# flanglet/kanzi-cpp

Hardware: AMD Instinct MI355X
Metric: encode+decode MB/s on the synthetic stand-in for silesia.tar (bit-exact) (higher is better)
Workload: dtype u8

## Files before the change

kanzi-cpp_amd/csrc/bwt_fwd.hip:

```cpp
#include "common.hpp"
#include "stages.hpp"
#include "bwt_common.hpp"

#include <cstdlib>
#include <cstring>
#include <algorithm>
#include <cmath>
#include "prims.hpp"
#include <chrono>
#include <vector>

namespace knz {

constexpr u32 SM_TS = 1792;
constexpr u32 SM_WIN = 2048;
constexpr u32 SM_G = 256;
constexpr u32 MED_CAP = 8192;
constexpr u32 SUPER_CAP = 8192;
constexpr int GATHER_THREADS = 512;
constexpr u32 LARGE_OS_MIN = 1000000;
constexpr u32 NO_BIT = 0x7FFFFFFFu;

struct FwdView {
    const u32* base;
// ... 1030 lines not shown
        if (mLab != oldLab) lab_set(v, gp, L.blkBase, mLab, oldLab);
    }
    u32 surv = 0;
    if (tid == 0) {
        if (less != 0) atomicOr(&v.gnew[mStart >> 5], 1u << (mStart & 31));
        if (c > SM_G) v.medStage[mStart >> 8] = make_uint2(mStart, c);
        else if (c > 1) surv = 1;
    }
    if ((u32)tid < nOth) {
        const u32 t = (u32)tid;
        const u32 key = L.oK[t];
        u32 hd = t, e = t + 1;
        while (hd > 0 && L.oK[hd - 1] == key) hd--;
        while (e < nOth && L.oK[e] == key) e++;
        const u32 size = e - hd;
        const u32 shift = (t < less) ? 0u : c;
        const u32 slot = gs + t + shift, hdSlot = gs + hd + shift;
        const u32 relO = rel - shift;
        const u32 lab = (size <= SM_G) ? hdSlot : ((oldLab >= hdSlot && oldLab < hdSlot + size) ? oldLab : hdSlot + (size >> 1));
        (void)relO;
        const u32 gp = L.oV[t];
        v.SA[slot] = gp;
        if (lab != oldLab) lab_set(v, gp, L.blkBase, lab, oldLab);
        if (t == hd) {
            if (hdSlot != gs) atomicOr(&v.gnew[hdSlot >> 5], 1u << (hdSlot & 31));
            if (size > SM_G) v.medStage[hdSlot >> 8] = make_uint2(hdSlot, size);
            else if (size > 1) surv = 1;
        }
    }
    if (__ballot(surv != 0) != 0 && (tid & 63) == 0) v.counters[0] = 1;
}

template <int THREADS, int ROWS>
__global__ __launch_bounds__(THREADS, (THREADS >= 1024 ? 4 : THREADS / 128)) void k_bwt_f_sort_medium(FwdView v, const uint2* __restrict__ desc, u32 nDesc, int npass, u32 minLen,
                                                               uint2* __restrict__ medNext, uint2* __restrict__ largeNext, const uint2* __restrict__ descInfo,
                                                               uint4* __restrict__ superList)
{
    constexpr int WAVES = THREADS / 64;
    constexpr u32 CAP = (u32)ROWS * THREADS;
    __shared__ MedLds<THREADS, ROWS> L;
    const int tid = (int)threadIdx.x, lane = tid & 63, wave = tid >> 6;
    const unsigned long long ltMask = (lane == 0) ? 0ull : (~0ull >> (64 - lane));

    for (u32 g = blockIdx.x; g < nDesc; g += gridDim.x) {
        const uint2 d = desc[g];
        const u32 gs = d.x, n = d.y;
        if (n <= minLen || n > CAP) continue;
        const uint2 info = descInfo[g];
        {
            u32 k[ROWS], p[ROWS];
#pragma unroll
            for (int r = 0; r < ROWS; r++) { const u32 i = (u32)tid + (u32)r * THREADS; k[r] = 0; p[r] = 0; if (i < n) { k[r] = v.K[gs + i]; p[r] = v.SA[gs + i]; } }
#pragma unroll
            for (int r = 0; r < ROWS; r++) { const u32 i = (u32)tid + (u32)r * THREADS; if (i < n) { L.oK[i] = k[r]; L.oV[i] = p[r]; } }
        }
        __syncthreads();
        if (tid == 0) { L.oldLab = info.y; L.blkBase = info.x; }
        const u32 ka = L.oK[n >> 2], kb = L.oK[n >> 1], kc = L.oK[(n >> 2) * 3];
        const u32 m = (ka == kc) ? ka : kb;
        u32 c = 0;
        for (u32 i = (u32)tid; i < n; i += THREADS) c += (L.oK[i] == m) ? 1u : 0u;
        c = med_block_sum(L, c);
        if (c < n && 2 * c >= n && n <= SUPER_CAP && m == info.y - info.x + 1u) {
            if (tid == 0) { const u32 at = atomicAdd(&v.counters[7], 1u); superList[at] = make_uint4(gs, n, info.x, info.y); }
            __syncthreads();
            continue;
        }
        if (c < n) {
            if (2 * c >= n) {
                const int R = (int)((n + THREADS - 1) / THREADS);
                const u32 waveBase = (u32)wave * (u32)R * 64u;
                u32 key[ROWS], val[ROWS], pos[ROWS];
                u32 runO = 0, runE = 0;
#pragma unroll
                for (int r = 0; r < ROWS; r++) {
                    key[r] = m; val[r] = 0; pos[r] = 0xFFFFFFFFu;
                    if (r < R) {
                        const u32 idx = waveBase + (u32)r * 64u + (u32)lane;
                        const bool valid = idx < n;
                        if (valid) { key[r] = L.oK[idx]; val[r] = L.oV[idx]; }
                        const bool oth = valid && key[r] != m, same = valid && key[r] == m;
                        const unsigned long long bo = __ballot(oth), be = __ballot(same);
                        if (oth) pos[r] = runO + (u32)__popcll(bo & ltMask);
                        if (same) pos[r] = 0x80000000u | (runE + (u32)__popcll(be & ltMask));
                        runO += (u32)__popcll(bo);
                        runE += (u32)__popcll(be);
                    }
                }
                if (lane == 0) { L.wtot[wave] = runO; L.wtot2[wave] = runE; }
                __syncthreads();
                u32 baseO = 0, baseE = 0, nOth = 0;
                for (int w = 0; w < WAVES; w++) { if (w < wave) { baseO += L.wtot[w]; baseE += L.wtot2[w]; } nOth += L.wtot[w]; }
#pragma unroll
                for (int r = 0; r < ROWS; r++) {
                    if (r < R && pos[r] != 0xFFFFFFFFu) {
                        const u32 at = (pos[r] & 0x80000000u) ? (nOth + baseE + (pos[r] & 0x7FFFFFFFu)) : (baseO + pos[r]);
                        L.oK[at] = key[r];
                        L.oV[at] = val[r];
                    }
                }
                __syncthreads();
                if (nOth <= (u32)THREADS) {
                    u32 kk = 0, vv = 0, at = 0;
                    if ((u32)tid < nOth) {
                        kk = L.oK[tid]; vv = L.oV[tid];
                        for (u32 j = 0; j < nOth; j++) { const u32 kj = L.oK[j]; at += (kj < kk || (kj == kk && j < (u32)tid)) ? 1u : 0u; }
                    }
                    __syncthreads();
                    if ((u32)tid < nOth) { L.oK[at] = kk; L.oV[at] = vv; }
                    __syncthreads();
                    u32 lessQ = 0;
                    if ((u32)tid < nOth) lessQ = (L.oK[tid] < m) ? 1u : 0u;
                    lessQ = med_block_sum(L, lessQ);
                    if (tid == 0) { L.oldLab = info.y; L.blkBase = info.x; }
                    __syncthreads();
                    med_majority_write_back<THREADS, ROWS>(L, v, gs, n, nOth, c, lessQ, m);
                    __syncthreads();
                    continue;
                } else {
                    med_radix_sort<THREADS, ROWS>(L, nOth, npass);
                }
                u32 less = 0;
                for (u32 i = (u32)tid; i < nOth; i += THREADS) less += (L.oK[i] < m) ? 1u : 0u;
                less = med_block_sum(L, less);
#pragma unroll
                for (int k = 0; k < ROWS; k++) {
                    const u32 i = (u32)tid + (u32)k * THREADS;
                    if (i < n) { key[k] = L.oK[i]; val[k] = L.oV[i]; }
                }
                __syncthreads();
#pragma unroll
                for (int k = 0; k < ROWS; k++) {
                    const u32 i = (u32)tid + (u32)k * THREADS;
                    if (i < n) {
                        const u32 at = (i < less) ? i : (i < nOth ? i + c : less + (i - nOth));
                        L.oK[at] = key[k];
                        L.oV[at] = val[k];
                    }
                }
                __syncthreads();
            } else {
                med_radix_sort<THREADS, ROWS>(L, n, npass);
            }
// ... 109 lines not shown
            cm = wave_max(cm);
            if (lane == 0 && cm) atomicMax(&sCmax, cm);
        }
        __syncthreads();
        const u32 cmax = sCmax;
        const u32 trBits = bitlen_u32(nEnds ? nEnds - 1 : 0), hiBits = bitlen_u32(2u * cmax + 1u);
        u32 fk[ROWS];
#pragma unroll
        for (int r = 0; r < ROWS; r++) {
            const u32 i = (u32)tid + (u32)r * THREADS;
            fk[r] = 0;
            if (i < n) { const u32 hiKey = (tail[r] < m) ? cc[r] : (2u * cmax + 1u - cc[r]); fk[r] = (hiKey << trBits) | (u32)trEnd[e[r]]; }
        }
        __syncthreads();
#pragma unroll
        for (int r = 0; r < ROWS; r++) { const u32 i = (u32)tid + (u32)r * THREADS; if (i < n) { L.oK[i] = fk[r]; L.oV[i] = i; } }
        __syncthreads();
        med_radix_sort<THREADS, ROWS>(L, n, (int)((hiBits + trBits + 7) / 8));
        {
            u32 p[ROWS];
#pragma unroll
            for (int r = 0; r < ROWS; r++) { const u32 i = (u32)tid + (u32)r * THREADS; p[r] = 0; if (i < n) p[r] = v.SA[gs + L.oV[i]]; }
            __syncthreads();
#pragma unroll
            for (int r = 0; r < ROWS; r++) { const u32 i = (u32)tid + (u32)r * THREADS; if (i < n) L.oV[i] = p[r]; }
        }
        __syncthreads();
        med_write_back<THREADS, ROWS>(L, v, gs, n, medNext, largeNext);
        __syncthreads();
    }
}

constexpr u32 PROBE_PMAX = 2048;
__global__ __launch_bounds__(256) void k_bwt_f_probe_scan(FwdView v, const uint2* __restrict__ desc, u32 depth, const u32* __restrict__ rtbits, u32* __restrict__ cand)
{
    const u32 nDesc = v.counters[1];
    for (u32 g = blockIdx.x * 256 + threadIdx.x; g < nDesc; g += gridDim.x * 256) {
        const uint2 d = desc[g];
        const u32 gs = d.x, n = d.y;
        if (n <= SM_G || n > SUPER_CAP) continue;
        if (rtbits != nullptr && ((rtbits[gs >> 5] >> (gs & 31)) & 1u)) continue;
        const u32 a0 = v.SA[gs + (n >> 1) - 2], a1 = v.SA[gs + (n >> 1) - 1], a2 = v.SA[gs + (n >> 1)], a3 = v.SA[gs + (n >> 1) + 1];
        const u32 pd = a2 - a1;
        if ((a1 - a0 == pd) && (a3 - a2 == pd) && (pd > depth) && (pd <= 2048u) && ((pd & (pd - 1)) != 0)) cand[atomicAdd(&v.counters[14], 1u)] = g;
    }
}

__global__ __launch_bounds__(512, 4) void k_bwt_f_probe(BwtView bv, FwdView v, uint2* __restrict__ desc, const u32* __restrict__ cand, u32 nCand, u32 depth, uint2* __restrict__ medNext,
                                                        uint2* __restrict__ largeNext, u32* __restrict__ ovr, u32* __restrict__ rtbits)
{
    constexpr int THREADS = 512, ROWS = 16;
    constexpr u32 CAP = (u32)ROWS * THREADS;
    __shared__ MedLds<THREADS, ROWS> L;
    __shared__ u32 patw[PROBE_PMAX / 4];
    u8* pat = reinterpret_cast<u8*>(patw);
    __shared__ u32 sInfo[4];
    const int tid = (int)threadIdx.x;
    for (u32 cg = blockIdx.x; cg < nCand; cg += gridDim.x) {
        const u32 g = cand[cg];
        const uint2 d = desc[g];
        const u32 gs = d.x, n = d.y;
        bool take = n > SM_G && n <= CAP;
        __syncthreads();
        if (take) {
            for (u32 i = (u32)tid; i < n; i += THREADS) L.oV[i] = v.SA[gs + i];
            if (tid == 0) {
                const int b = find_block(v.base, v.nBlocks, gs);
                sInfo[0] = v.base[b]; sInfo[1] = v.base[b + 1]; sInfo[3] = (u32)b;
            }
        }
        __syncthreads();
        u32 P = 0, pr = 0;
        if (take) {
            pr = L.oV[n >> 1];
            P = pr - L.oV[(n >> 1) - 1];
            take = P > depth && P <= PROBE_PMAX && pr + P <= sInfo[1];
        }
        if (take) {
            u32 c = 0;
            for (u32 i = (u32)tid; i + 1 < n; i += THREADS) c += (L.oV[i + 1] - L.oV[i] == P) ? 1u : 0u;
            c = med_block_sum(L, c);
            take = 2 * c >= n;
        }
        if (!take) continue;
        const u32 bb = sInfo[0], be = sInfo[1];
        const u8* t = bv.src[sInfo[3]];
        for (u32 j = (u32)tid; j < P; j += THREADS) pat[j] = ldg<u8>(t + (pr - bb + j));
        if (tid == 0) sInfo[2] = lab_cur(v, pr, sInfo[0]);
        __syncthreads();
        constexpr u32 MID = 1u << 21;
        u32 nEq = 0, nBelow = 0;
        for (u32 i = (u32)tid; i < n; i += THREADS) {
            const u32 q0 = L.oV[i] - bb;
            u32 l = depth;
            if ((depth & 3u) == 0) {
                const u32* pw = patw;
                while (l + 16 <= P && q0 + l + 20 <= be - bb) {
                    const uintptr_t ad = reinterpret_cast<uintptr_t>(t + q0 + l);
                    const u8* w = reinterpret_cast<const u8*>(ad & ~(uintptr_t)3);
                    const u32 sh = (u32)(ad & 3) * 8;
                    const u32 w0 = ldg<u32>(w), w1 = ldg<u32>(w + 4), w2 = ldg<u32>(w + 8), w3 = ldg<u32>(w + 12), w4 = ldg<u32>(w + 16);
                    const u32 x0 = sh ? ((w0 >> sh) | (w1 << (32 - sh))) : w0, x1 = sh ? ((w1 >> sh) | (w2 << (32 - sh))) : w1;
                    const u32 x2 = sh ? ((w2 >> sh) | (w3 << (32 - sh))) : w2, x3 = sh ? ((w3 >> sh) | (w4 << (32 - sh))) : w3;
                    const u32 d0 = x0 ^ pw[l >> 2], d1 = x1 ^ pw[(l >> 2) + 1], d2 = x2 ^ pw[(l >> 2) + 2], d3 = x3 ^ pw[(l >> 2) + 3];
                    if ((d0 | d1 | d2 | d3) != 0) break;
                    l += 16;
                }
            }
            u32 code = MID;
            while (l < P) {
                if (q0 + l >= be - bb) { code = l * 512u; break; }
                const u32 x = ldg<u8>(t + q0 + l), y = pat[l];
                if (x != y) { code = (x < y) ? (l * 512u + x + 1u) : (MID + 1u + (P - l) * 512u + x + 1u); break; }
                l++;
            }
            L.oK[i] = code;
            nEq += (code == MID) ? 1u : 0u;
            nBelow += (code < MID) ? 1u : 0u;
        }
        nEq = med_block_sum(L, nEq);
        nBelow = med_block_sum(L, nBelow);
        if (2 * nEq < n) continue;
        if (tid == 0) { L.oldLab = sInfo[2]; L.blkBase = sInfo[0]; desc[g].y = 0; }
        med_radix_sort<THREADS, ROWS>(L, n, 3);
        med_write_back<THREADS, ROWS>(L, v, gs, n, medNext, largeNext);
        for (u32 i = (u32)tid; i < n; i += THREADS) {
            const u32 code = L.oK[i];
            const u32 lshare = (code == MID) ? P : ((code < MID) ? (code >> 9) : (P - ((code - MID - 1u) >> 9))) + 1u;
            ovr[gs + i] = lshare;
            atomicOr(&rtbits[(gs + i) >> 5], 1u << ((gs + i) & 31));
        }
    }
}

__global__ __launch_bounds__(1024) void k_bwt_f_large_prefix(const uint2* __restrict__ desc, u32 nDesc, u32* __restrict__ loff, const u32* __restrict__ base, int nBlocks,
                                                             u32* __restrict__ lbase)
{
    __shared__ u32 part[1024];
    const u32 per = (nDesc + 1023) / 1024;
    const u32 lo = threadIdx.x * per, hi = (lo + per < nDesc) ? lo + per : nDesc;
    u32 sum = 0;
    for (u32 i = lo; i < hi; i++) { sum += desc[i].y; lbase[i] = base[find_block(base, nBlocks, desc[i].x)]; }
    part[threadIdx.x] = sum;
    __syncthreads();
    if (threadIdx.x == 0) { u32 run = 0; for (int t = 0; t < 1024; t++) { const u32 x = part[t]; part[t] = run; run += x; } loff[nDesc] = run; }
    __syncthreads();
    u32 run = part[threadIdx.x];
    for (u32 i = lo; i < hi; i++) { loff[i] = run; run += desc[i].y; }
}

template <class KEY>
__global__ __launch_bounds__(256) void k_bwt_f_large_keys(FwdView v, const uint2* __restrict__ desc, u32 nDesc, const u32* __restrict__ loff,
                                                          u32 L, u32 h, int kbits, KEY* __restrict__ keys, u32* __restrict__ vals)
{
    const u32 j = blockIdx.x * 256 + threadIdx.x;
    if (j >= L) return;
    u32 lo = 0, hi = nDesc;
    while (hi - lo > 1) { const u32 mid = (lo + hi) >> 1; if (loff[mid] <= j) lo = mid; else hi = mid; }
    const uint2 d = desc[lo];
    const u32 slot = d.x + (j - loff[lo]);
    const int b = find_block(v.base, v.nBlocks, d.x);
    const u32 gp = v.SA[slot];
    u32 off = h;
// ... 398 lines not shown
            const u32 q = 4 * w + k;
            if (q >= qLo && q < qHi) {
                const u32 rr = q - qLo;
                const u32 r = rr + (rr >= r0 ? 1u : 0u);
                const u32 p = SA[bb + r] - bb;
                word |= (u32)s[p - 1] << (8 * k);
                have |= 1u << k;
            }
        }
        if (have == 0xF && al) reinterpret_cast<u32*>(d)[w] = word;
        else for (u32 k = 0; k < 4; k++) if ((have >> k) & 1) d[4 * w + k] = (u8)(word >> (8 * k));
    }
    if (blockIdx.x == 0 && threadIdx.x == 0) {
        d[hdr] = s[n - 1];
        const u32 st = n / (u32)chunks;
        const u32 step = ((u32)chunks * st == n) ? st : st + 1;
        const u32 logNbChunks = (u32)ilog2_u32((u32)chunks);
        d[0] = (u8)((logNbChunks << 2) | (pIndexSize - 1));
        u32 idx = 1;
        for (int k = 0; k < chunks; k++) {
            const u32 prim = lab_cur(fv, bb + (u32)k * step, bb) - bb;
            for (int sh = (int)(pIndexSize - 1) * 8; sh >= 0; sh -= 8) d[idx++] = (u8)(prim >> sh);
        }
        newLen[b] = hdr + n;
    }
}

__global__ __launch_bounds__(256) void k_bwt_f_med_flags(const uint2* __restrict__ stage, u32 nSlots, u32* __restrict__ flags)
{
    const u32 i = blockIdx.x * 256 + threadIdx.x;
    if (i < nSlots) flags[i] = stage[i].y ? 1u : 0u;
}

__global__ __launch_bounds__(256) void k_bwt_f_med_compact(uint2* __restrict__ stage, u32 nSlots, const u32* __restrict__ prefix, uint2* __restrict__ medNext)
{
    const u32 i = blockIdx.x * 256 + threadIdx.x;
    if (i >= nSlots) return;
    const uint2 d = stage[i];
    if (d.y) { medNext[prefix[i]] = d; stage[i] = make_uint2(0u, 0u); }
}

struct FwdTuning { int nsym; int noRunRound; int runFallback; int stats; int link; int plainLabels; int noPack; };
static FwdTuning& fwd_tuning()
{
    static FwdTuning t = [] {
        FwdTuning x; x.nsym = 0; x.noRunRound = 0; x.runFallback = 0; x.stats = 0; x.link = 1; x.plainLabels = 0; x.noPack = 0;
        if (getenv("KNZ_BWT_PLAIN_LABELS")) x.plainLabels = 1;
        if (getenv("KNZ_BWT_NO_PACK")) x.noPack = 1;
        if (const char* e = getenv("KNZ_BWT_LINK")) x.link = atoi(e);
        if (getenv("KNZ_BWT_STATS")) x.stats = 1;
        if (const char* e = getenv("KNZ_BWT_NSYM")) x.nsym = atoi(e);
        if (getenv("KNZ_BWT_NO_RUN_ROUND")) x.noRunRound = 1;
        if (getenv("KNZ_BWT_RUN_FALLBACK")) x.runFallback = 1;
        return x;
    }();
    return t;
}
int bwt_forward_tune(const char* key, int value)
{
    FwdTuning& t = fwd_tuning();
    if (!strcmp(key, "rs_onesweep")) { prims::rs_onesweep_knob().store(value); return 0; }
    if (!strcmp(key, "bwt_nsym")) t.nsym = value;
    else if (!strcmp(key, "bwt_no_run_round")) t.noRunRound = value;
    else if (!strcmp(key, "bwt_run_fallback")) t.runFallback = value;
    else if (!strcmp(key, "bwt_stats")) t.stats = value;
    else if (!strcmp(key, "bwt_link")) t.link = value;
// ... 138 lines not shown
        std::swap(kin, kout);
    }
    const u64* sortedKeys = kin;
    u64* keysFree = kout;
    u64* keysFree2 = const_cast<u64*>(sortedKeys);
    hipMemsetAsync(w.gbits, 0xFF, 4 * w.gbitsWords, s);
    hipMemsetAsync(w.gnew, 0, 4 * w.gbitsWords, s);
    hipMemsetAsync(w.counters, 0, 64, s);
    { KScope ks_("k_bwt_f_r0_flags"); hipLaunchKernelGGL(k_bwt_f_r0_flags, dim3((total + 256 * R0F_ROWS - 1) / (256 * R0F_ROWS)), dim3(256), 0, s, sortedKeys, w.base, st.nBlocks, total, nsym, pbits,
                                                         reinterpret_cast<unsigned long long*>(w.gbits)); }
    const u32 nWinP = (total + SM_TS - 1) / SM_TS;
    { KScope ks_("k_bwt_f_r0_winsum"); hipLaunchKernelGGL(k_bwt_f_r0_winsum, GRID1(nWinP), w.gbits, total, nWinP, w.t0, w.t2, SM_TS / 32); }
    { KScope ks_("k_bwt_f_scan_max"); prims::launch_scan<prims::SCAN_MAX_INCL>(s, w.t0, w.t1, nWinP, nullptr, w.scanTmp); }
    { KScope ks_("k_bwt_f_scan_min"); prims::launch_scan<prims::SCAN_MIN_INCL>(s, w.t2, w.t3, nWinP, nullptr, w.scanTmp); }
    int cur = 0;
    int kbits = 1;
    while ((1ull << kbits) < (u64)bv.VS + 2) kbits++;
    const bool runRound = (2 * kbits + 1) < 64 && !tune.noRunRound;
    { KScope ks_("k_bwt_f_r0_place");
      hipLaunchKernelGGL(k_bwt_f_r0_place_text, dim3(nWinP), dim3(256), 0, s, bv, v, w.t1, w.t3, nWinP, w.large[cur], sortedKeys, nsym, pbits, runRound ? w.runList : (uint2*)nullptr);
      hipLaunchKernelGGL(k_bwt_f_merge_bits, GRID1(total / 32 + 2), w.gbits, w.gnew, total / 32 + 2); }
    if (hipMemcpyAsync(h_pinned, w.counters, 64, hipMemcpyDeviceToHost, s) != hipSuccess) return -1;
    if (hipStreamSynchronize(s) != hipSuccess) return -1;
    u32 nRun = h_pinned[4], runElems = h_pinned[5];
    bool medCompacted = false;
    const int maxKeyBits = 2 * kbits + 1;
    if (nRun && ((u64)nRun > (1ull << (64 - maxKeyBits)) || tune.runFallback)) {
        { KScope ks_("k_bwt_f_run_fallback"); hipLaunchKernelGGL(k_bwt_f_run_fallback, GRID1(nRun), v, w.runList, nRun, w.med[cur], w.large[cur]); }
        if (hipMemcpyAsync(h_pinned, w.counters, 64, hipMemcpyDeviceToHost, s) != hipSuccess) return -1;
        if (hipStreamSynchronize(s) != hipSuccess) return -1;
        nRun = 0;
    }
    u32* probeCand = w.medFlags;
    auto probeScan = [&]() {
        KScope ks_("k_bwt_f_probe");
        hipLaunchKernelGGL(k_bwt_f_probe_scan, dim3(256), dim3(256), 0, s, v, w.med[cur], (u32)nsym, v.rtbits, probeCand);
    };
    prims::RsWs rs1 = prims::rs_carve(w.rsMem, maxTotal, st.nBlocks + 1, w.seg2, 1);
    if (nRun) {
        const u32 nWin = (total + SM_WIN - 1) / SM_WIN;
        { KScope ks_("k_bwt_f_run_ends"); hipLaunchKernelGGL(k_bwt_f_run_ends, dim3((total + SM_WIN - 1) / SM_WIN), dim3(256), 0, s, bv, v, reinterpret_cast<u8*>(w.ebits)); }
        { KScope ks_("k_bwt_f_r0_winsum"); hipLaunchKernelGGL(k_bwt_f_r0_winsum, GRID1(nWin), w.ebits, total, nWin, w.t0, w.t2, SM_WIN / 32); }
        { KScope ks_("k_bwt_f_scan_min"); prims::launch_scan<prims::SCAN_MIN_INCL>(s, w.t2, w.t3, nWin, nullptr, w.scanTmp); }
        hipMemsetAsync(w.classTab, 0xFF, 1024ull * (size_t)st.nBlocks, s);
        { KScope ks_("k_bwt_f_run_classes"); hipLaunchKernelGGL(k_bwt_f_run_classes, GRID1(nRun), bv, v, w.runList, nRun, w.classTab); }
        { KScope ks_("k_bwt_f_run_len"); hipLaunchKernelGGL(k_bwt_f_run_len, dim3(nWin), dim3(256), 0, s, bv, v, w.ebits, w.t3, nWin, w.K, w.classTab, (u32)nsym,
                                                            reinterpret_cast<unsigned long long*>(w.rbits), w.rcount); }
        const u32 nRW = nWin * (SM_WIN / 32);
        { KScope ks_("k_bwt_f_scan_sum"); prims::launch_scan<prims::SCAN_SUM_EXCL>(s, w.rcount, w.rprefix, nRW, nullptr, w.scanTmp, w.counters + 8); }
        { KScope ks_("k_bwt_f_run_compact"); hipLaunchKernelGGL(k_bwt_f_run_compact, GRID1(nRW), w.rbits, w.rprefix, nRW, w.runPos); }
        if (hipMemcpyAsync(h_pinned + 8, w.counters + 6, 12, hipMemcpyDeviceToHost, s) != hipSuccess) return -1;
        if (hipStreamSynchronize(s) != hipSuccess) return -1;
        const u32 nRuns = h_pinned[10];
        int hbits = 1;
        while ((1ull << hbits) < (u64)h_pinned[8] + 1) hbits++;
        hbits++;
        const int keyBits = hbits + kbits;
        int rbits = 0;
        while ((1u << rbits) < nRun) rbits++;
        int idxBits = 1;
        while ((1ull << idxBits) < (u64)nRuns) idxBits++;
        if (nRuns == 0 || nRuns > w.maxRuns || rbits + hbits > 32 || idxBits + kbits + 1 + rbits > 64) {
            { KScope ks_("k_bwt_f_run_fallback"); hipLaunchKernelGGL(k_bwt_f_run_fallback, GRID1(nRun), v, w.runList, nRun, w.med[cur], w.large[cur]); }
            if (hipMemcpyAsync(h_pinned, w.counters, 64, hipMemcpyDeviceToHost, s) != hipSuccess) return -1;
            if (hipStreamSynchronize(s) != hipSuccess) return -1;
            nRun = 0;
        }
      if (nRun) {
        { KScope ks_("k_bwt_f_large_prefix"); hipLaunchKernelGGL(k_bwt_f_large_prefix, dim3(1), dim3(1024), 0, s, w.runList, nRun, w.loff, w.base, st.nBlocks, w.lbase); }
// ... 17 lines not shown
          rk = r ? keysFree : keysFree2;
          hipLaunchKernelGGL(k_bwt_f_run_expand, GRID1(runElems), sortedM, runElems, w.sKey, w.sE, kbits, hbits, rk, rv, w.valsB); }
        {
            u32* mbits = w.ebits;
            const u32 nWinM = (runElems + SM_WIN - 1) / SM_WIN;
            { KScope ks_("k_bwt_f_large_flags"); hipLaunchKernelGGL(k_bwt_f_run_flags, dim3(nWinM * (SM_WIN / 256)), dim3(256), 0, s, rk, runElems, reinterpret_cast<unsigned long long*>(mbits)); }
            { KScope ks_("k_bwt_f_r0_winsum"); hipLaunchKernelGGL(k_bwt_f_r0_winsum, GRID1(nWinM), mbits, runElems, nWinM, w.t0, w.t2, SM_WIN / 32); }
            { KScope ks_("k_bwt_f_scan_max"); prims::launch_scan<prims::SCAN_MAX_INCL>(s, w.t0, w.t1, nWinM, nullptr, w.scanTmp); }
            { KScope ks_("k_bwt_f_scan_min"); prims::launch_scan<prims::SCAN_MIN_INCL>(s, w.t2, w.t3, nWinM, nullptr, w.scanTmp); }
            { KScope ks_("k_bwt_f_large_place");
              hipMemsetAsync(w.rtbits, 0, 4 * w.gbitsWords, s);
              hipLaunchKernelGGL(k_bwt_f_run_place, dim3((runElems + 255) / 256), dim3(256), 0, s, v, w.runList, w.loff, runElems, keyBits, rk, rv, mbits, w.t1, w.t3, nWinM, w.large[cur],
                                 w.valsB, w.ovr, w.rtbits, w.lbase);
              v.ovr = w.ovr; v.rtbits = w.rtbits; }
        }
        { KScope ks_("k_bwt_f_merge_bits"); hipLaunchKernelGGL(k_bwt_f_merge_bits, GRID1(total / 32 + 2), w.gbits, w.gnew, total / 32 + 2); }
        compactMedium(w.med[cur]);
        probeScan();
        medCompacted = true;
        if (hipMemcpyAsync(h_pinned, w.counters, 64, hipMemcpyDeviceToHost, s) != hipSuccess) return -1;
        if (hipStreamSynchronize(s) != hipSuccess) return -1;
      }
    }
    if (!medCompacted) {
        compactMedium(w.med[cur]);
        probeScan();
        if (hipMemcpyAsync(h_pinned, w.counters, 64, hipMemcpyDeviceToHost, s) != hipSuccess) return -1;
        if (hipStreamSynchronize(s) != hipSuccess) return -1;
    }
    u32 surv = h_pinned[0], nMed = h_pinned[1], nLarge = h_pinned[2], largeElems = h_pinned[3];
    if (const u32 nCand = h_pinned[14]) {
        if (!v.rtbits) { hipMemsetAsync(w.rtbits, 0, 4 * w.gbitsWords, s); v.ovr = w.ovr; v.rtbits = w.rtbits; }
        hipMemsetAsync(w.counters, 0, 8, s);
        { KScope ks_("k_bwt_f_probe");
          hipLaunchKernelGGL(k_bwt_f_probe, dim3(std::min<u32>(nCand, 4096)), dim3(512), 0, s, bv, v, w.med[cur], probeCand, nCand, (u32)nsym, w.med[cur ^ 1], w.large[cur], w.ovr, w.rtbits);
          hipLaunchKernelGGL(k_bwt_f_merge_bits, GRID1(total / 32 + 2), w.gbits, w.gnew, total / 32 + 2); }
        compactMedium(w.med[cur] + nMed);
        if (hipMemcpyAsync(h_pinned, w.counters, 8, hipMemcpyDeviceToHost, s) != hipSuccess) return -1;
        if (hipStreamSynchronize(s) != hipSuccess) return -1;
        surv |= h_pinned[0];
        nMed += h_pinned[1];
    }
    if (tune.stats) fprintf(stderr, "after round 0 (nsym %d, total %u): run groups %u (%u members); small left %u, medium %u, large %u (%u members)\n",
                            nsym, total, nRun, runElems, surv, nMed, nLarge, largeElems);
    std::chrono::steady_clock::time_point statT = std::chrono::steady_clock::now();

    const int npass = (kbits + 7) / 8;
    const u32 nTiles = (total + SM_TS - 1) / SM_TS;
    u32 h = 1;
    while (2 * h <= (u32)nsym) h <<= 1;
    u32 survMembers = total;
    int linkMode = 0;
    u32 linkStepUsed = 1, linkRetryH = 0xFFFFFFFFu;
    LinkTrial linkTr; linkTr.n = 0;
    int linkTrials = 0;
    while (surv || nMed || nLarge) {
        if (h > bv.VS) return -5;
        { KScope ks_("k_bwt_f_round"); hipMemsetAsync(w.counters, 0, 64, s); }
        v.round++;
        if (v.round > 255) return -5;
        const int nxt = cur ^ 1;
        bool linkNow = false;
        u32 linkStep = 1;
        if (surv && tune.link && h >= (u32)(tune.link > 1 ? tune.link : 32)) {
            if (linkMode == 1 || linkMode == 3) {
                const u32 linkedN = h_pinned[14], tiedN = h_pinned[15];
                const bool paid = linkedN >= 4096 && tiedN < linkedN / 2;
                linkMode = paid ? 2 : 4;
                if (!paid) linkRetryH = (linkTrials < 2) ? h * 8 : 0xFFFFFFFFu;
                if (tune.stats) fprintf(stderr, "link step: %u members linked, %u of the windows' members still tied after the round -> %s\n", linkedN, tiedN, paid ? "on" : "off");
            }
            if (linkMode == 4 && h >= linkRetryH) linkMode = 0;
            if (linkMode == 0 && survMembers >= total / 8) { linkNow = true; linkMode = 1; linkTrials++; }
            else if (linkMode == 2 && survMembers >= total / 64) { linkNow = true; linkMode = 3; }
// ... 110 lines not shown
```

Baseline: 5645.

## Use periodic mismatch bitmaps to link probe positions and skip redundant comparisons

The probe scan now builds a small table of frequent periods found across medium groups. For common periods it precomputes per-position bitmaps of mismatches between text[j] and text[j+P]. The probe kernel then links each suffix to its predecessor at distance P and resolves comparison codes through chains, instead of comparing every suffix against the pattern byte by byte. It also adds a few-outliers path (split majority plus rank sort instead of radix), word-level rtbits writes, and restaging of the medium list. The costs are an extra bitmap kernel, scratch memory reuse, and more complex control flow.

```diff
diff --git a/kanzi-cpp_amd/csrc/bwt_fwd.hip b/kanzi-cpp_amd/csrc/bwt_fwd.hip
--- a/kanzi-cpp_amd/csrc/bwt_fwd.hip
+++ b/kanzi-cpp_amd/csrc/bwt_fwd.hip
@@ -1086,15 +1086,68 @@
 }
 
 template <int THREADS, int ROWS>
+__device__ __forceinline__ u32 med_split_majority(MedLds<THREADS, ROWS>& L, u32 n, u32 m, u32 (&key)[ROWS], u32 (&val)[ROWS])
+{
+    constexpr int WAVES = THREADS / 64;
+    const int lane = (int)threadIdx.x & 63, wave = (int)threadIdx.x >> 6;
+    const unsigned long long ltMask = (lane == 0) ? 0ull : (~0ull >> (64 - lane));
+    const int R = (int)((n + THREADS - 1) / THREADS);
+    const u32 waveBase = (u32)wave * (u32)R * 64u;
+    u32 pos[ROWS];
+    u32 runO = 0, runE = 0;
+#pragma unroll
+    for (int r = 0; r < ROWS; r++) {
+        key[r] = m; val[r] = 0; pos[r] = 0xFFFFFFFFu;
+        if (r < R) {
+            const u32 idx = waveBase + (u32)r * 64u + (u32)lane;
+            const bool valid = idx < n;
+            if (valid) { key[r] = L.oK[idx]; val[r] = L.oV[idx]; }
+            const bool oth = valid && key[r] != m, same = valid && key[r] == m;
+            const unsigned long long bo = __ballot(oth), be = __ballot(same);
+            if (oth) pos[r] = runO + (u32)__popcll(bo & ltMask);
+            if (same) pos[r] = 0x80000000u | (runE + (u32)__popcll(be & ltMask));
+            runO += (u32)__popcll(bo);
+            runE += (u32)__popcll(be);
+        }
+    }
+    if (lane == 0) { L.wtot[wave] = runO; L.wtot2[wave] = runE; }
+    __syncthreads();
+    u32 baseO = 0, baseE = 0, nOth = 0;
+    for (int w = 0; w < WAVES; w++) { if (w < wave) { baseO += L.wtot[w]; baseE += L.wtot2[w]; } nOth += L.wtot[w]; }
+#pragma unroll
+    for (int r = 0; r < ROWS; r++) {
+        if (r < R && pos[r] != 0xFFFFFFFFu) {
+            const u32 at = (pos[r] & 0x80000000u) ? (nOth + baseE + (pos[r] & 0x7FFFFFFFu)) : (baseO + pos[r]);
+            L.oK[at] = key[r];
+            L.oV[at] = val[r];
+        }
+    }
+    __syncthreads();
+    return nOth;
+}
+
+template <int THREADS, int ROWS>
+__device__ __forceinline__ void med_rank_few(MedLds<THREADS, ROWS>& L, u32 k)
+{
+    const int tid = (int)threadIdx.x;
+    u32 kk = 0, vv = 0, at = 0;
+    if ((u32)tid < k) {
+        kk = L.oK[tid]; vv = L.oV[tid];
+        for (u32 j = 0; j < k; j++) { const u32 kj = L.oK[j]; at += (kj < kk || (kj == kk && j < (u32)tid)) ? 1u : 0u; }
+    }
+    __syncthreads();
+    if ((u32)tid < k) { L.oK[at] = kk; L.oV[at] = vv; }
+    __syncthreads();
+}
+
+template <int THREADS, int ROWS>
 __global__ __launch_bounds__(THREADS, (THREADS >= 1024 ? 4 : THREADS / 128)) void k_bwt_f_sort_medium(FwdView v, const uint2* __restrict__ desc, u32 nDesc, int npass, u32 minLen,
                                                                uint2* __restrict__ medNext, uint2* __restrict__ largeNext, const uint2* __restrict__ descInfo,
                                                                uint4* __restrict__ superList)
 {
-    constexpr int WAVES = THREADS / 64;
     constexpr u32 CAP = (u32)ROWS * THREADS;
     __shared__ MedLds<THREADS, ROWS> L;
-    const int tid = (int)threadIdx.x, lane = tid & 63, wave = tid >> 6;
-    const unsigned long long ltMask = (lane == 0) ? 0ull : (~0ull >> (64 - lane));
+    const int tid = (int)threadIdx.x;
 
     for (u32 g = blockIdx.x; g < nDesc; g += gridDim.x) {
         const uint2 d = desc[g];
@@ -1122,47 +1175,10 @@
         }
         if (c < n) {
             if (2 * c >= n) {
-                const int R = (int)((n + THREADS - 1) / THREADS);
-                const u32 waveBase = (u32)wave * (u32)R * 64u;
-                u32 key[ROWS], val[ROWS], pos[ROWS];
-                u32 runO = 0, runE = 0;
-#pragma unroll
-                for (int r = 0; r < ROWS; r++) {
-                    key[r] = m; val[r] = 0; pos[r] = 0xFFFFFFFFu;
-                    if (r < R) {
-                        const u32 idx = waveBase + (u32)r * 64u + (u32)lane;
-                        const bool valid = idx < n;
-                        if (valid) { key[r] = L.oK[idx]; val[r] = L.oV[idx]; }
-                        const bool oth = valid && key[r] != m, same = valid && key[r] == m;
-                        const unsigned long long bo = __ballot(oth), be = __ballot(same);
-                        if (oth) pos[r] = runO + (u32)__popcll(bo & ltMask);
-                        if (same) pos[r] = 0x80000000u | (runE + (u32)__popcll(be & ltMask));
-                        runO += (u32)__popcll(bo);
-                        runE += (u32)__popcll(be);
-                    }
-                }
-                if (lane == 0) { L.wtot[wave] = runO; L.wtot2[wave] = runE; }
-                __syncthreads();
-                u32 baseO = 0, baseE = 0, nOth = 0;
-                for (int w = 0; w < WAVES; w++) { if (w < wave) { baseO += L.wtot[w]; baseE += L.wtot2[w]; } nOth += L.wtot[w]; }
-#pragma unroll
-                for (int r = 0; r < ROWS; r++) {
-                    if (r < R && pos[r] != 0xFFFFFFFFu) {
-                        const u32 at = (pos[r] & 0x80000000u) ? (nOth + baseE + (pos[r] & 0x7FFFFFFFu)) : (baseO + pos[r]);
-                        L.oK[at] = key[r];
-                        L.oV[at] = val[r];
-                    }
-                }
-                __syncthreads();
+                u32 key[ROWS], val[ROWS];
+                const u32 nOth = med_split_majority<THREADS, ROWS>(L, n, m, key, val);
                 if (nOth <= (u32)THREADS) {
-                    u32 kk = 0, vv = 0, at = 0;
-                    if ((u32)tid < nOth) {
-                        kk = L.oK[tid]; vv = L.oV[tid];
-                        for (u32 j = 0; j < nOth; j++) { const u32 kj = L.oK[j]; at += (kj < kk || (kj == kk && j < (u32)tid)) ? 1u : 0u; }
-                    }
-                    __syncthreads();
-                    if ((u32)tid < nOth) { L.oK[at] = kk; L.oV[at] = vv; }
-                    __syncthreads();
+                    med_rank_few<THREADS, ROWS>(L, nOth);
                     u32 lessQ = 0;
                     if ((u32)tid < nOth) lessQ = (L.oK[tid] < m) ? 1u : 0u;
                     lessQ = med_block_sum(L, lessQ);
@@ -1338,22 +1354,109 @@
 }
 
 constexpr u32 PROBE_PMAX = 2048;
-__global__ __launch_bounds__(256) void k_bwt_f_probe_scan(FwdView v, const uint2* __restrict__ desc, u32 depth, const u32* __restrict__ rtbits, u32* __restrict__ cand)
+constexpr u32 PROBE_NP = 8;
+__device__ __forceinline__ u32 probe_period(const u32* pos, u32 n, u32 depth, u32& m)
+{
+    const u32 at[3] = {n >> 1, (n >> 1) + 2u, (n >> 1) - 3u};
+    for (int k = 0; k < 3; k++) {
+        const u32 i = at[k];
+        const u32 a0 = pos[i - 2], a1 = pos[i - 1], a2 = pos[i], a3 = pos[i + 1];
+        const u32 pd = a2 - a1;
+        if (a1 - a0 == pd && a3 - a2 == pd && pd > depth && pd <= PROBE_PMAX) { m = i; return pd; }
+    }
+    return 0;
+}
+
+__global__ __launch_bounds__(256) void k_bwt_f_probe_scan(FwdView v, const uint2* __restrict__ desc, u32 depth, const u32* __restrict__ rtbits, u32* __restrict__ cand,
+                                                          u32* __restrict__ ptab)
 {
     const u32 nDesc = v.counters[1];
-    for (u32 g = blockIdx.x * 256 + threadIdx.x; g < nDesc; g += gridDim.x * 256) {
-        const uint2 d = desc[g];
-        const u32 gs = d.x, n = d.y;
-        if (n <= SM_G || n > SUPER_CAP) continue;
-        if (rtbits != nullptr && ((rtbits[gs >> 5] >> (gs & 31)) & 1u)) continue;
-        const u32 a0 = v.SA[gs + (n >> 1) - 2], a1 = v.SA[gs + (n >> 1) - 1], a2 = v.SA[gs + (n >> 1)], a3 = v.SA[gs + (n >> 1) + 1];
-        const u32 pd = a2 - a1;
-        if ((a1 - a0 == pd) && (a3 - a2 == pd) && (pd > depth) && (pd <= 2048u) && ((pd & (pd - 1)) != 0)) cand[atomicAdd(&v.counters[14], 1u)] = g;
-    }
+    for (u32 g0 = blockIdx.x * 256; g0 < nDesc; g0 += gridDim.x * 256) {
+        const u32 g = g0 + threadIdx.x;
+        u32 pd = 0, n = 0;
+        if (g < nDesc) {
+            const uint2 d = desc[g];
+            const u32 gs = d.x;
+            n = d.y;
+            u32 m;
+            if (n > SM_G && n <= SUPER_CAP && !(rtbits != nullptr && ((rtbits[gs >> 5] >> (gs & 31)) & 1u)))
+                pd = probe_period(v.SA + gs, n, depth, m);
+        }
+        int slot = -1;
+        if (pd != 0) {
+            u32 e[PROBE_NP];
+#pragma unroll
+            for (u32 k = 0; k < PROBE_NP; k++) e[k] = __atomic_load_n(&ptab[k], __ATOMIC_RELAXED);
+#pragma unroll
+            for (u32 k = 0; k < PROBE_NP; k++) if (slot < 0 && e[k] == pd) slot = (int)k;
+            for (u32 k = 0; k < PROBE_NP && slot < 0; k++) {
+                if (e[k] != 0u) continue;
+                const u32 o = atomicCAS(&ptab[k], 0u, pd);
+                if (o == 0u || o == pd) slot = (int)k;
+            }
+        }
+        for (u32 k = 0; k < PROBE_NP; k++) {
+            const u32 sum = wave_sum(slot == (int)k ? n : 0u);
+            if ((threadIdx.x & 63) == 0 && sum) atomicAdd(&ptab[PROBE_NP + k], sum);
+        }
+        if (pd != 0 && (slot >= 0 || (pd & (pd - 1)) != 0)) cand[atomicAdd(&v.counters[14], 1u)] = g;
+    }
+}
+
+__device__ __forceinline__ u32 nonzero_bytes(u32 x)
+{
+    const u32 hb = (((x & 0x7F7F7F7Fu) + 0x7F7F7F7Fu) | x) & 0x80808080u;
+    return ((hb >> 7) & 1u) | ((hb >> 14) & 2u) | ((hb >> 21) & 4u) | ((hb >> 28) & 8u);
+}
+
+__device__ __forceinline__ void load32_unaligned(const u8* p, u32 (&x)[8])
+{
+    const uintptr_t ad = reinterpret_cast<uintptr_t>(p);
+    const u8* w = reinterpret_cast<const u8*>(ad & ~(uintptr_t)3);
+    const u32 sh = (u32)(ad & 3) * 8;
+    u32 r[9];
+#pragma unroll
+    for (int k = 0; k < 8; k++) r[k] = ldg<u32>(w + 4 * k);
+    r[8] = sh ? ldg<u32>(w + 32) : 0u;
+#pragma unroll
+    for (int k = 0; k < 8; k++) x[k] = sh ? ((r[k] >> sh) | (r[k + 1] << (32 - sh))) : r[k];
+}
+
+__device__ __forceinline__ bool probe_has_map(const u32* __restrict__ ptab, u32 k, u32 total) { return ptab[k] != 0u && ptab[PROBE_NP + k] >= total / 256u; }
+
+__global__ __launch_bounds__(256) void k_bwt_f_probe_dbits(BwtView bv, FwdView v, const u32* __restrict__ ptab, u32* __restrict__ dbits, u32 nWords)
+{
+    if (!probe_has_map(ptab, blockIdx.y, v.total)) return;
+    const u32 P = ptab[blockIdx.y];
+    const u32 w = blockIdx.x * 256 + threadIdx.x;
+    if (w >= nWords) return;
+    u32* out = dbits + (size_t)blockIdx.y * nWords;
+    const u32 j0 = w * 32u;
+    if (j0 >= v.total) { out[w] = 0xFFFFFFFFu; return; }
+    int b = find_block(v.base, v.nBlocks, j0);
+    u32 bb = v.base[b], be = v.base[b + 1];
+    const u8* t = bv.src[b];
+    u32 bits = 0;
+    if (j0 + 32u + P <= be) {
+        u32 a[8], c[8];
+        load32_unaligned(t + (j0 - bb), a);
+        load32_unaligned(t + (j0 - bb) + P, c);
+#pragma unroll
+        for (int k = 0; k < 8; k++) bits |= nonzero_bytes(a[k] ^ c[k]) << (4 * k);
+    } else {
+        for (u32 k = 0; k < 32; k++) {
+            const u32 j = j0 + k;
+            if (j >= v.total) { bits |= 0xFFFFFFFFu << k; break; }
+            while (j >= be) { b++; bb = be; be = v.base[b + 1]; t = bv.src[b]; }
+            if (j + P >= be || ldg<u8>(t + (j - bb)) != ldg<u8>(t + (j - bb + P))) bits |= 1u << k;
+        }
+    }
+    out[w] = bits;
 }
 
 __global__ __launch_bounds__(512, 4) void k_bwt_f_probe(BwtView bv, FwdView v, uint2* __restrict__ desc, const u32* __restrict__ cand, u32 nCand, u32 depth, uint2* __restrict__ medNext,
-                                                        uint2* __restrict__ largeNext, u32* __restrict__ ovr, u32* __restrict__ rtbits)
+                                                        uint2* __restrict__ largeNext, u32* __restrict__ ovr, u32* __restrict__ rtbits, const u32* __restrict__ ptab,
+                                                        const u32* __restrict__ dbits, u32 nWords)
 {
     constexpr int THREADS = 512, ROWS = 16;
     constexpr u32 CAP = (u32)ROWS * THREADS;
@@ -1361,6 +1464,8 @@
     __shared__ u32 patw[PROBE_PMAX / 4];
     u8* pat = reinterpret_cast<u8*>(patw);
     __shared__ u32 sInfo[4];
+    __shared__ u32 sMoved[2];
+    __shared__ u32 sHeads, sTake;
     const int tid = (int)threadIdx.x;
     for (u32 cg = blockIdx.x; cg < nCand; cg += gridDim.x) {
         const u32 g = cand[cg];
@@ -1368,6 +1473,15 @@
         const u32 gs = d.x, n = d.y;
         bool take = n > SM_G && n <= CAP;
         __syncthreads();
+        if (take && tid == 0) {
+            u32 m0;
+            const u32 P0 = probe_period(v.SA + gs, n, depth, m0);
+            bool ok = P0 != 0 && (P0 & (P0 - 1)) != 0;
+            for (u32 k = 0; k < PROBE_NP && !ok; k++) ok = dbits != nullptr && ptab[k] == P0 && probe_has_map(ptab, k, v.total);
+            sTake = ok ? 1u : 0u;
+        }
+        __syncthreads();
+        take = take && sTake != 0;
         if (take) {
             for (u32 i = (u32)tid; i < n; i += THREADS) L.oV[i] = v.SA[gs + i];
             if (tid == 0) {
@@ -1378,48 +1492,173 @@
         __syncthreads();
         u32 P = 0, pr = 0;
         if (take) {
-            pr = L.oV[n >> 1];
-            P = pr - L.oV[(n >> 1) - 1];
-            take = P > depth && P <= PROBE_PMAX && pr + P <= sInfo[1];
-        }
+            u32 m = 0;
+            P = probe_period(L.oV, n, depth, m);
+            pr = L.oV[m];
+            take = P != 0 && pr + P <= sInfo[1];
+        }
+        const u32* dP = nullptr;
         if (take) {
-            u32 c = 0;
-            for (u32 i = (u32)tid; i + 1 < n; i += THREADS) c += (L.oV[i + 1] - L.oV[i] == P) ? 1u : 0u;
+            u32 c = 0, unsorted = 0;
+            for (u32 i = (u32)tid; i + 1 < n; i += THREADS) {
+                c += (L.oV[i + 1] - L.oV[i] == P) ? 1u : 0u;
+                unsorted += (L.oV[i + 1] <= L.oV[i]) ? 1u : 0u;
+            }
             c = med_block_sum(L, c);
+            unsorted = med_block_sum(L, unsorted);
             take = 2 * c >= n;
+            if (unsorted == 0 && dbits != nullptr)
+                for (u32 k = 0; k < PROBE_NP; k++) if (ptab[k] == P && probe_has_map(ptab, k, v.total)) dP = dbits + (size_t)k * nWords;
+            if (dP == nullptr && (P & (P - 1)) == 0) take = false;
         }
         if (!take) continue;
         const u32 bb = sInfo[0], be = sInfo[1];
         const u8* t = bv.src[sInfo[3]];
         for (u32 j = (u32)tid; j < P; j += THREADS) pat[j] = ldg<u8>(t + (pr - bb + j));
         if (tid == 0) sInfo[2] = lab_cur(v, pr, sInfo[0]);
-        __syncthreads();
-        constexpr u32 MID = 1u << 21;
-        u32 nEq = 0, nBelow = 0;
-        for (u32 i = (u32)tid; i < n; i += THREADS) {
-            const u32 q0 = L.oV[i] - bb;
-            u32 l = depth;
-            if ((depth & 3u) == 0) {
-                const u32* pw = patw;
-                while (l + 16 <= P && q0 + l + 20 <= be - bb) {
-                    const uintptr_t ad = reinterpret_cast<uintptr_t>(t + q0 + l);
-                    const u8* w = reinterpret_cast<const u8*>(ad & ~(uintptr_t)3);
-                    const u32 sh = (u32)(ad & 3) * 8;
-                    const u32 w0 = ldg<u32>(w), w1 = ldg<u32>(w + 4), w2 = ldg<u32>(w + 8), w3 = ldg<u32>(w + 12), w4 = ldg<u32>(w + 16);
-                    const u32 x0 = sh ? ((w0 >> sh) | (w1 << (32 - sh))) : w0, x1 = sh ? ((w1 >> sh) | (w2 << (32 - sh))) : w1;
-                    const u32 x2 = sh ? ((w2 >> sh) | (w3 << (32 - sh))) : w2, x3 = sh ? ((w3 >> sh) | (w4 << (32 - sh))) : w3;
-                    const u32 d0 = x0 ^ pw[l >> 2], d1 = x1 ^ pw[(l >> 2) + 1], d2 = x2 ^ pw[(l >> 2) + 2], d3 = x3 ^ pw[(l >> 2) + 3];
-                    if ((d0 | d1 | d2 | d3) != 0) break;
-                    l += 16;
+        u32 nLinked = 0;
+        if (dP) {
+            u32 acc[ROWS];
+#pragma unroll
+            for (int r = 0; r < ROWS; r++) {
+                const u32 i = (u32)tid + (u32)r * THREADS;
+                acc[r] = 0;
+                if (i >= n) continue;
+                L.oK[i] = i;
+                const u32 p = L.oV[i];
+                if (i == 0 || p - bb < P) continue;
+                const u32 q = p - P;
+                u32 j = i - 1;
+                if (L.oV[j] != q) {
+                    u32 lo = 0, hi = i;
+                    while (lo < hi) { const u32 mid = (lo + hi) >> 1; if (L.oV[mid] < q) lo = mid + 1; else hi = mid; }
+                    j = lo;
+                }
+                if (j < i && L.oV[j] == q) L.oK[i] = j;
+            }
+            const u32 nw = (P + 31) / 32 + 1;
+            for (u32 k = 0; k < nw; k++) {
+#pragma unroll
+                for (int r = 0; r < ROWS; r++) {
+                    const u32 i = (u32)tid + (u32)r * THREADS;
+                    if (i >= n || L.oK[i] == i) continue;
+                    const u32 p = L.oV[i], q = p - P;
+                    const u32 w = (q >> 5) + k;
+                    if (w > ((p - 1) >> 5)) continue;
+                    u32 x = dP[w];
+                    if (k == 0) x &= 0xFFFFFFFFu << (q & 31);
+                    if (w == ((p - 1) >> 5) && (p & 31)) x &= 0xFFFFFFFFu >> (32 - (p & 31));
+                    acc[r] |= x;
                 }
             }
-            u32 code = MID;
-            while (l < P) {
-                if (q0 + l >= be - bb) { code = l * 512u; break; }
-                const u32 x = ldg<u8>(t + q0 + l), y = pat[l];
-                if (x != y) { code = (x < y) ? (l * 512u + x + 1u) : (MID + 1u + (P - l) * 512u + x + 1u); break; }
-                l++;
+#pragma unroll
+            for (int r = 0; r < ROWS; r++) {
+                const u32 i = (u32)tid + (u32)r * THREADS;
+                if (i >= n) continue;
+                if (acc[r]) L.oK[i] = i;
+                nLinked += (L.oK[i] != i) ? 1u : 0u;
             }
+            nLinked = med_block_sum(L, nLinked);
+        }
+        if (nLinked) {
+            for (u32 it = 0;; it ^= 1) {
+                u32 a[ROWS];
+                bool moved = false;
+#pragma unroll
+                for (int r = 0; r < ROWS; r++) {
+                    const u32 i = (u32)tid + (u32)r * THREADS;
+                    a[r] = 0;
+                    if (i < n) { const u32 j = L.oK[i]; a[r] = L.oK[j]; moved = moved || (a[r] != j); }
+                }
+                if (tid == 0) sMoved[it] = 0;
+                __syncthreads();
+                if (moved) sMoved[it] = 1;
+#pragma unroll
+                for (int r = 0; r < ROWS; r++) { const u32 i = (u32)tid + (u32)r * THREADS; if (i < n) L.oK[i] = a[r]; }
+                __syncthreads();
+                if (!sMoved[it]) break;
+            }
+        }
+        __syncthreads();
+        constexpr u32 MID = 1u << 21, HEAD = 0x80000000u;
+        const u32 nHeads = n - nLinked;
+        if (nLinked && nHeads <= (u32)(THREADS / 64) * 256u) {
+            const int lane = tid & 63, wave = tid >> 6;
+            if (tid == 0) sHeads = 0;
+            __syncthreads();
+#pragma unroll
+            for (int r = 0; r < ROWS; r++) {
+                const u32 i = (u32)tid + (u32)r * THREADS;
+                if (i < n && L.oK[i] == i) L.cnt[atomicAdd(&sHeads, 1u)] = i;
+            }
+            __syncthreads();
+            for (u32 h = (u32)wave; h < nHeads; h += (u32)(THREADS / 64)) {
+                const u32 i = L.cnt[h];
+                const u32 q0 = L.oV[i] - bb, len = be - bb;
+                u32 code = MID;
+                for (u32 l0 = depth; l0 < P; l0 += 256) {
+                    constexpr u32 NONE = 0xFFFFFFFFu;
+                    u32 x[4];
+#pragma unroll
+                    for (int e = 0; e < 4; e++) { const u32 l = l0 + (u32)lane * 4u + (u32)e; x[e] = (l < P && q0 + l < len) ? (u32)ldg<u8>(t + q0 + l) : 0u; }
+                    u32 ev = NONE;
+#pragma unroll
+                    for (int e = 3; e >= 0; e--) {
+                        const u32 l = l0 + (u32)lane * 4u + (u32)e;
+                        if (l < P && (q0 + l >= len || x[e] != pat[l])) ev = l;
+                    }
+                    const unsigned long long bal = __ballot(ev != NONE);
+                    if (bal) {
+                        const u32 l = (u32)__shfl((int)ev, __ffsll((long long)bal) - 1, 64);
+                        if (q0 + l >= len) code = l * 512u;
+                        else {
+                            const u32 xb = ldg<u8>(t + q0 + l), y = pat[l];
+                            code = (xb < y) ? (l * 512u + xb + 1u) : (MID + 1u + (P - l) * 512u + xb + 1u);
+                        }
+                        break;
+                    }
+                }
+                if (lane == 0) L.oK[i] = code | HEAD;
+            }
+        } else {
+#pragma unroll
+            for (int r = 0; r < ROWS; r++) {
+                const u32 i = (u32)tid + (u32)r * THREADS;
+                if (i >= n || (nLinked && L.oK[i] != i)) continue;
+                const u32 q0 = L.oV[i] - bb;
+                u32 l = depth;
+                if ((depth & 3u) == 0) {
+                    const u32* pw = patw;
+                    while (l + 16 <= P && q0 + l + 20 <= be - bb) {
+                        const uintptr_t ad = reinterpret_cast<uintptr_t>(t + q0 + l);
+                        const u8* w = reinterpret_cast<const u8*>(ad & ~(uintptr_t)3);
+                        const u32 sh = (u32)(ad & 3) * 8;
+                        const u32 w0 = ldg<u32>(w), w1 = ldg<u32>(w + 4), w2 = ldg<u32>(w + 8), w3 = ldg<u32>(w + 12), w4 = ldg<u32>(w + 16);
+                        const u32 x0 = sh ? ((w0 >> sh) | (w1 << (32 - sh))) : w0, x1 = sh ? ((w1 >> sh) | (w2 << (32 - sh))) : w1;
+                        const u32 x2 = sh ? ((w2 >> sh) | (w3 << (32 - sh))) : w2, x3 = sh ? ((w3 >> sh) | (w4 << (32 - sh))) : w3;
+                        const u32 d0 = x0 ^ pw[l >> 2], d1 = x1 ^ pw[(l >> 2) + 1], d2 = x2 ^ pw[(l >> 2) + 2], d3 = x3 ^ pw[(l >> 2) + 3];
+                        if ((d0 | d1 | d2 | d3) != 0) break;
+                        l += 16;
+                    }
+                }
+                u32 code = MID;
+                while (l < P) {
+                    if (q0 + l >= be - bb) { code = l * 512u; break; }
+                    const u32 x = ldg<u8>(t + q0 + l), y = pat[l];
+                    if (x != y) { code = (x < y) ? (l * 512u + x + 1u) : (MID + 1u + (P - l) * 512u + x + 1u); break; }
+                    l++;
+                }
+                L.oK[i] = code | HEAD;
+            }
+        }
+        __syncthreads();
+        u32 nEq = 0, nBelow = 0;
+#pragma unroll
+        for (int r = 0; r < ROWS; r++) {
+            const u32 i = (u32)tid + (u32)r * THREADS;
+            if (i >= n) continue;
+            const u32 x = L.oK[i];
+            const u32 code = ((x & HEAD) ? x : L.oK[x]) & ~HEAD;
             L.oK[i] = code;
             nEq += (code == MID) ? 1u : 0u;
             nBelow += (code < MID) ? 1u : 0u;
@@ -1427,14 +1666,34 @@
         nEq = med_block_sum(L, nEq);
         nBelow = med_block_sum(L, nBelow);
         if (2 * nEq < n) continue;
-        if (tid == 0) { L.oldLab = sInfo[2]; L.blkBase = sInfo[0]; desc[g].y = 0; }
-        med_radix_sort<THREADS, ROWS>(L, n, 3);
-        med_write_back<THREADS, ROWS>(L, v, gs, n, medNext, largeNext);
+        if (tid == 0) {
+            L.oldLab = sInfo[2]; L.blkBase = sInfo[0]; desc[g].y = 0;
+            atomicAdd(&v.counters[34], 1u);
+            if (nLinked) atomicAdd(&v.counters[35], 1u);
+            if (nLinked && nHeads > (u32)(THREADS / 64) * 256u) atomicAdd(&v.counters[36], 1u);
+        }
+        const u32 nOth = n - nEq;
+        const bool few = nOth <= (u32)THREADS;
+        if (few) {
+            u32 key[ROWS], val[ROWS];
+            med_split_majority<THREADS, ROWS>(L, n, MID, key, val);
+            med_rank_few<THREADS, ROWS>(L, nOth);
+            med_majority_write_back<THREADS, ROWS>(L, v, gs, n, nOth, nEq, nBelow, MID);
+        } else {
+            med_radix_sort<THREADS, ROWS>(L, n, 3);
+            med_write_back<THREADS, ROWS>(L, v, gs, n, medNext, largeNext);
+        }
         for (u32 i = (u32)tid; i < n; i += THREADS) {
-            const u32 code = L.oK[i];
+            const u32 code = !few ? L.oK[i] : (i < nBelow ? L.oK[i] : (i < nBelow + nEq ? MID : L.oK[i - nEq]));
             const u32 lshare = (code == MID) ? P : ((code < MID) ? (code >> 9) : (P - ((code - MID - 1u) >> 9))) + 1u;
             ovr[gs + i] = lshare;
-            atomicOr(&rtbits[(gs + i) >> 5], 1u << ((gs + i) & 31));
+        }
+        for (u32 w = (gs >> 5) + (u32)tid; w <= (gs + n - 1) >> 5; w += THREADS) {
+            u32 mask = 0xFFFFFFFFu;
+            if (w == (gs >> 5)) mask &= 0xFFFFFFFFu << (gs & 31);
+            if (w == ((gs + n - 1) >> 5)) mask &= 0xFFFFFFFFu >> (31 - ((gs + n - 1) & 31));
+            if (mask == 0xFFFFFFFFu) rtbits[w] = mask;
+            else atomicOr(&rtbits[w], mask);
         }
     }
 }
@@ -1899,6 +2158,13 @@
     if (i < nSlots) flags[i] = stage[i].y ? 1u : 0u;
 }
 
+__global__ __launch_bounds__(256) void k_bwt_f_med_restage(const uint2* __restrict__ list, u32 n, uint2* __restrict__ stage)
+{
+    const u32 i = blockIdx.x * 256 + threadIdx.x;
+    if (i >= n) return;
+    const uint2 d = list[i];
+    if (d.y) stage[d.x >> 8] = d;
+}
 __global__ __launch_bounds__(256) void k_bwt_f_med_compact(uint2* __restrict__ stage, u32 nSlots, const u32* __restrict__ prefix, uint2* __restrict__ medNext)
 {
     const u32 i = blockIdx.x * 256 + threadIdx.x;
@@ -2103,9 +2369,11 @@
         nRun = 0;
     }
     u32* probeCand = w.medFlags;
+    u32* probeTab = w.counters + 16;
     auto probeScan = [&]() {
         KScope ks_("k_bwt_f_probe");
-        hipLaunchKernelGGL(k_bwt_f_probe_scan, dim3(256), dim3(256), 0, s, v, w.med[cur], (u32)nsym, v.rtbits, probeCand);
+        hipMemsetAsync(probeTab, 0, 8 * PROBE_NP, s);
+        hipLaunchKernelGGL(k_bwt_f_probe_scan, dim3(256), dim3(256), 0, s, v, w.med[cur], (u32)nsym, v.rtbits, probeCand, probeTab);
     };
     prims::RsWs rs1 = prims::rs_carve(w.rsMem, maxTotal, st.nBlocks + 1, w.seg2, 1);
     if (nRun) {
@@ -2189,14 +2457,29 @@
     if (const u32 nCand = h_pinned[14]) {
         if (!v.rtbits) { hipMemsetAsync(w.rtbits, 0, 4 * w.gbitsWords, s); v.ovr = w.ovr; v.rtbits = w.rtbits; }
         hipMemsetAsync(w.counters, 0, 8, s);
+        hipMemsetAsync(w.counters + 34, 0, 12, s);
+        const u32 nWords = (total + 31) / 32 + 1;
+        u32* dbits = (size_t)PROBE_NP * nWords * 4 <= 8ull * total ? reinterpret_cast<u32*>(keysFree) : (u32*)nullptr;
+        if (dbits) { KScope ks_("k_bwt_f_probe_dbits"); hipLaunchKernelGGL(k_bwt_f_probe_dbits, dim3((nWords + 255) / 256, PROBE_NP), dim3(256), 0, s, bv, v, probeTab, dbits, nWords); }
         { KScope ks_("k_bwt_f_probe");
-          hipLaunchKernelGGL(k_bwt_f_probe, dim3(std::min<u32>(nCand, 4096)), dim3(512), 0, s, bv, v, w.med[cur], probeCand, nCand, (u32)nsym, w.med[cur ^ 1], w.large[cur], w.ovr, w.rtbits);
+          hipLaunchKernelGGL(k_bwt_f_probe, dim3(std::min<u32>(nCand, 4096)), dim3(512), 0, s, bv, v, w.med[cur], probeCand, nCand, (u32)nsym, w.med[cur ^ 1], w.large[cur], w.ovr, w.rtbits,
+                             probeTab, dbits, nWords);
           hipLaunchKernelGGL(k_bwt_f_merge_bits, GRID1(total / 32 + 2), w.gbits, w.gnew, total / 32 + 2); }
-        compactMedium(w.med[cur] + nMed);
+        { KScope ks_("k_bwt_f_med_compact"); hipLaunchKernelGGL(k_bwt_f_med_restage, GRID1(nMed), w.med[cur], nMed, w.medStage); }
+        compactMedium(w.med[cur]);
         if (hipMemcpyAsync(h_pinned, w.counters, 8, hipMemcpyDeviceToHost, s) != hipSuccess) return -1;
         if (hipStreamSynchronize(s) != hipSuccess) return -1;
         surv |= h_pinned[0];
-        nMed += h_pinned[1];
+        nMed = h_pinned[1];
+        if (tune.stats) {
+            const u32* c = h_pinned + 64;
+            if (hipMemcpyAsync(h_pinned + 64, w.counters + 16, 96, hipMemcpyDeviceToHost, s) != hipSuccess) return -1;
+            if (hipStreamSynchronize(s) != hipSuccess) return -1;
+            u32 nP = 0, nMaps = 0;
+            for (u32 k = 0; k < PROBE_NP; k++) { nP += c[k] != 0u; nMaps += (dbits != nullptr && c[k] != 0u && c[PROBE_NP + k] >= total / 256u); }
+            fprintf(stderr, "probe: %u candidates, %u periods in the table (%u with a bit map); %u groups taken, %u by stretch (%u with many heads)\n",
+                    nCand, nP, nMaps, c[18], c[19], c[20]);
+        }
     }
     if (tune.stats) fprintf(stderr, "after round 0 (nsym %d, total %u): run groups %u (%u members); small left %u, medium %u, large %u (%u members)\n",
                             nsym, total, nRun, runElems, surv, nMed, nLarge, largeElems);
```

After: 6012, median of 6. +6.5%, better.
